# JoshuaLim007/VoxelEngine

Hardware: AMD Instinct MI355X
Metric: Mrays/s primary+1-bounce @1080p, 8k×512×8k brickmap; % HBM roofline (higher is better)
Workload: dtype f32

## Files before the change

include/vxrt.h:

```cpp
#ifndef VXRT_H
#define VXRT_H

#include <stddef.h>
#include <stdint.h>

#ifdef __cplusplus
extern "C" {
#endif

#define VXRT_ABI_VERSION 3
#define VXRT_EMPTY_SLOT 0xFFFFFFFFu
#define VXRT_MAX_STEPS 2048

typedef enum vxrt_status {
    VXRT_OK = 0,
    VXRT_ERR_INVALID = -1,
    VXRT_ERR_HIP = -2,
    VXRT_ERR_NO_WORLD = -3,
    VXRT_ERR_NOMEM = -4
} vxrt_status;

typedef struct vxrt_ctx vxrt_ctx;

int vxrt_abi_version(void);
// ... 318 lines not shown
    int32_t bounce_all_hits;
    int32_t bounce_depth;
    int32_t ortho;
    int64_t frame_number;
    int32_t strip_rows, strip_count, strip_index;
    int32_t compact;
    int32_t collect_stats;
    int32_t tile_schedule;
    float *d_color_aov;
    int64_t *d_hit_aov;
    const uint32_t *d_tile_order;
    void *stream;
    float *d_accum;
    int32_t accum_reset;
    int32_t reserved_;
} vxrt_render_flags;

void vxrt_render_flags_default(vxrt_render_flags *flags);
int vxrt_render(vxrt_ctx *ctx, uint32_t width, uint32_t height, void *d_fb, const float origin[3],
                const float fwd[3], const float up[3], const float right[3], const vxrt_render_flags *flags);
typedef struct vxrt_view {
    void *d_fb;
    float origin[3], fwd[3], up[3], right[3];
    int64_t frame_number;
    float *d_color_aov;
    int64_t *d_hit_aov;
} vxrt_view;
int vxrt_render_views(vxrt_ctx *ctx, uint32_t width, uint32_t height, uint32_t n_views, const vxrt_view *views,
                      const vxrt_render_flags *flags);
int vxrt_kernel_for_launch(const vxrt_ctx *ctx, uint32_t width, uint32_t height, const vxrt_render_flags *flags, uint32_t nviews);
int vxrt_render_specialisation(const vxrt_ctx *ctx, uint32_t width, uint32_t height, const vxrt_render_flags *flags, uint32_t nviews);
uint32_t vxrt_compact_rows(uint32_t height, int32_t strip_rows, int32_t strip_count, int32_t strip_index);
int vxrt_frame_stats_get(vxrt_ctx *ctx, vxrt_frame_stats *out);
int vxrt_deinterleave_strips(vxrt_ctx *ctx, uint32_t width, uint32_t height, int32_t strip_rows,
                             int32_t strip_count, const void *d_shards, uint64_t shard_stride_bytes,
                             void *d_fb, void *stream);
int vxrt_deinterleave_views(vxrt_ctx *ctx, uint32_t width, uint32_t height, int32_t strip_rows, int32_t strip_count,
                            const void *d_shards, uint64_t shard_stride_bytes, uint64_t view_stride_bytes,
                            uint32_t n_views, void *d_fb, uint64_t fb_stride_bytes, void *stream);

typedef struct vxrt_denoise_params {
    uint32_t struct_size;
    int32_t iterations;
    float color_scale;
    int32_t reserved_;
} vxrt_denoise_params;
int vxrt_frame_guides(vxrt_ctx *ctx, uint32_t W, uint32_t H, const float origin[3], const float fwd[3], const float up[3],
                      const float right[3], int32_t ortho, const int64_t *d_hit_aov, uint32_t *d_keys, void *stream);
uint64_t vxrt_denoise_workspace_bytes(uint32_t W, uint32_t H);
int vxrt_denoise_frame(vxrt_ctx *ctx, uint32_t W, uint32_t H, const float *d_color_in , const uint32_t *d_keys,
                       const vxrt_denoise_params *params, void *d_work, float *d_color_out ,
                       void *d_fb_or_null , void *stream);

typedef struct vxrt_history { float r, g, b, n; } vxrt_history;
typedef struct vxrt_camera_pose { float origin[3], fwd[3], up[3], right[3]; } vxrt_camera_pose;
typedef struct vxrt_reproject_params {
    uint32_t struct_size;
    int32_t ortho;
    int32_t max_history;
    int32_t reserved_;
    vxrt_camera_pose cur, prev;
} vxrt_reproject_params;
typedef struct vxrt_reproject_summary { uint32_t hit, reused, offscreen, rejected; } vxrt_reproject_summary;
int vxrt_reproject_frame(vxrt_ctx *ctx, uint32_t W, uint32_t H, const float *d_color_in, const uint32_t *d_keys,
                         const vxrt_history *d_hist_in_or_null, const uint32_t *d_keys_prev_or_null,
                         const vxrt_reproject_params *params, vxrt_history *d_hist_out,
// ... 36 lines not shown
```

voxelengine_amd/_native.py:

```python
from __future__ import annotations

import ctypes as C
import os

from . import build as _build

EMPTY_SLOT = 0xFFFFFFFF
MAX_STEPS = 2048
GEN_HASH_HEIGHTFIELD, GEN_PERLIN_REF, GEN_INT_TERRAIN = 0, 1, 2
MODE_SHADED, MODE_DEBUG = 0, 1

EXPORTS = [
    "vxrt_abi_version", "vxrt_create", "vxrt_destroy", "vxrt_last_error", "vxrt_synchronize", "vxrt_set_kernel_variant", "vxrt_kernel_for_launch",
    "vxrt_render_specialisation",
    "vxrt_has_experiments", "vxrt_set_persistent_waves_per_cu", "vxrt_debug_guard_pretend_no_slack",
    "vxrt_upload_world", "vxrt_build_world_procedural", "vxrt_world_info_get", "vxrt_download_world",
    "vxrt_save_world", "vxrt_load_world", "vxrt_world_file_info",
    "vxrt_set_environment", "vxrt_set_fov", "vxrt_set_ortho_window_size", "vxrt_get_directions",
    "vxrt_render_flags_default", "vxrt_render", "vxrt_render_views", "vxrt_compact_rows", "vxrt_frame_stats_get",
    "vxrt_deinterleave_strips", "vxrt_deinterleave_views", "vxrt_trace_batch", "vxrt_trace_batch_host",
    "vxrt_set_batch_max_steps", "vxrt_stream_open", "vxrt_stream_focus", "vxrt_stream_resident", "vxrt_stream_close",
    "vxrt_edit_voxels", "vxrt_edit_reserve",
    "vxrt_region_words", "vxrt_read_region", "vxrt_read_region_host", "vxrt_edit_stamps",
    "vxrt_move_boxes", "vxrt_overlap_boxes", "vxrt_move_boxes_host", "vxrt_overlap_boxes_host",
    "vxrt_islands_workspace_bytes", "vxrt_find_islands", "vxrt_find_islands_host",
    "vxrt_place_pieces", "vxrt_place_pieces_host",
    "vxrt_orientation_rotation", "vxrt_orientation_compose", "vxrt_orientation_inverse", "vxrt_orientation_dims",
    "vxrt_orientation_voxel", "vxrt_orientation_is_rotation", "vxrt_transform_stamp", "vxrt_transform_stamp_host",
    "vxrt_nav_workspace_bytes", "vxrt_nav_field", "vxrt_nav_paths", "vxrt_nav_field_host",
    "vxrt_distance_workspace_bytes", "vxrt_distance_field", "vxrt_distance_field_host",
    "vxrt_voxelize_workspace_bytes", "vxrt_voxelize_mesh", "vxrt_voxelize_mesh_host",
    "vxrt_surface_workspace_bytes", "vxrt_extract_surface", "vxrt_extract_surface_host",
    "vxrt_lod_workspace_bytes", "vxrt_downsample_region", "vxrt_downsample_region_host",
    "vxrt_light_workspace_bytes", "vxrt_light_field", "vxrt_light_field_host",
    "vxrt_rule_workspace_bytes", "vxrt_apply_rule", "vxrt_apply_rule_host",
    "vxrt_frame_guides", "vxrt_denoise_workspace_bytes", "vxrt_denoise_frame", "vxrt_reproject_frame", "vxrt_light_frame",
]
EDIT_BOX, EDIT_SPHERE = 0, 1
EDIT_MAX_OPS = 1024
STAMP_REPLACE, STAMP_UNION, STAMP_SUBTRACT = 0, 1, 2
BODY_MAX_EXTENT, BODY_MAX_DELTA = 64, 64
BODY_BLOCKED_X, BODY_BLOCKED_Y, BODY_BLOCKED_Z, BODY_INVALID = 1, 2, 4, 8
ISLAND_ANCHOR_X_LO, ISLAND_ANCHOR_X_HI, ISLAND_ANCHOR_Y_LO, ISLAND_ANCHOR_Y_HI = 0x01, 0x02, 0x04, 0x08
ISLAND_ANCHOR_Z_LO, ISLAND_ANCHOR_Z_HI, ISLAND_ANCHOR_FACES, ISLAND_ANCHOR_FLOOR = 0x10, 0x20, 0x3F, 0x40
PLACE_MAX_PIECES, PLACE_MAX_DIM, PLACE_MAX_VOXELS, PLACE_MAX_DIST = 64, 1024, 1 << 24, 4096
PLACED_BLOCKED, PLACED_INVALID = 1, 2
NAV_MAX_GOALS, NAV_NONE, NAV_MAX_STEPS = 4096, 0xFF, 65535
NAV_AT_GOAL, NAV_NO_PATH, NAV_TRUNCATED, NAV_OUTSIDE = 0, 1, 2, 3
DIST_TO_SOLID, DIST_TO_EMPTY, DIST_FAR, DIST_MAX_RADIUS = 0, 1, 0xFFFF, 255
VOX_SURFACE, VOX_SOLID, VOX_FRAC_BITS, VOX_MAX_DIM, VOX_MAX_COORD, VOX_MAX_TRIANGLES = 1, 2, 8, 1024, 1 << 18, 1 << 24
SURF_CAP, SURF_OPEN, SURF_MAX_DIM = 0, 1, 1024
LOD_MAX_SHIFT = 5
# ... 132 lines not shown
    f3 = C.POINTER(C.c_float)
    L.vxrt_abi_version.restype = C.c_int
    L.vxrt_last_error.restype = C.c_char_p
    L.vxrt_create.argtypes = [C.c_int, C.POINTER(C.c_void_p)]
    L.vxrt_destroy.argtypes = [C.c_void_p]
    L.vxrt_synchronize.argtypes = [C.c_void_p]
    L.vxrt_set_kernel_variant.argtypes = [C.c_void_p, C.c_int]
    L.vxrt_has_experiments.restype = C.c_int
    L.vxrt_debug_guard_pretend_no_slack.argtypes = [C.c_void_p, C.c_int]
    L.vxrt_set_persistent_waves_per_cu.argtypes = [C.c_void_p, C.c_int]
    L.vxrt_kernel_for_launch.argtypes = [C.c_void_p, C.c_uint32, C.c_uint32, C.c_void_p, C.c_uint32]
    L.vxrt_kernel_for_launch.restype = C.c_int
    L.vxrt_render_specialisation.argtypes = [C.c_void_p, C.c_uint32, C.c_uint32, C.c_void_p, C.c_uint32]
    L.vxrt_render_specialisation.restype = C.c_int
    L.vxrt_upload_world.argtypes = [C.c_void_p, C.POINTER(WorldDesc)]
    L.vxrt_build_world_procedural.argtypes = [C.c_void_p, C.c_int, C.c_int, C.c_int, C.c_int, C.c_int]
    L.vxrt_world_info_get.argtypes = [C.c_void_p, C.POINTER(WorldInfo)]
    L.vxrt_download_world.argtypes = [C.c_void_p, C.c_void_p, C.c_void_p, C.c_void_p, C.c_void_p]
    L.vxrt_save_world.argtypes = [C.c_void_p, C.c_char_p]
    L.vxrt_load_world.argtypes = [C.c_void_p, C.c_char_p]
    L.vxrt_world_file_info.argtypes = [C.c_char_p, C.POINTER(WorldInfo)]
    L.vxrt_set_environment.argtypes = [C.c_void_p, f3, f3, f3]
    L.vxrt_set_fov.argtypes = [C.c_void_p, C.c_float]
    L.vxrt_set_ortho_window_size.argtypes = [C.c_void_p, C.c_float, C.c_float]
    L.vxrt_get_directions.argtypes = [f3, f3, f3, f3]
    L.vxrt_get_directions.restype = None
    L.vxrt_render_flags_default.argtypes = [C.POINTER(RenderFlags)]
    L.vxrt_render_flags_default.restype = None
    L.vxrt_render.argtypes = [C.c_void_p, C.c_uint32, C.c_uint32, C.c_void_p, f3, f3, f3, f3, C.POINTER(RenderFlags)]
    L.vxrt_render_views.argtypes = [C.c_void_p, C.c_uint32, C.c_uint32, C.c_uint32, C.POINTER(View), C.POINTER(RenderFlags)]
    L.vxrt_compact_rows.argtypes = [C.c_uint32, C.c_int32, C.c_int32, C.c_int32]
    L.vxrt_compact_rows.restype = C.c_uint32
    L.vxrt_frame_stats_get.argtypes = [C.c_void_p, C.POINTER(FrameStats)]
    L.vxrt_deinterleave_strips.argtypes = [C.c_void_p, C.c_uint32, C.c_uint32, C.c_int32, C.c_int32, C.c_void_p,
                                           C.c_uint64, C.c_void_p, C.c_void_p]
    L.vxrt_deinterleave_views.argtypes = [C.c_void_p, C.c_uint32, C.c_uint32, C.c_int32, C.c_int32, C.c_void_p, C.c_uint64,
                                          C.c_uint64, C.c_uint32, C.c_void_p, C.c_uint64, C.c_void_p]
    L.vxrt_trace_batch.argtypes = [C.c_void_p, C.c_void_p, C.c_void_p, C.c_uint64, C.c_void_p, C.c_void_p, C.c_void_p,
                                   C.c_void_p, C.c_void_p, C.POINTER(FrameStats), C.c_void_p]
    L.vxrt_set_batch_max_steps.argtypes = [C.c_void_p, C.c_int32]
    L.vxrt_stream_open.argtypes = [C.c_void_p, C.c_char_p, C.c_uint64]
    L.vxrt_stream_focus.argtypes = [C.c_void_p, f3, C.c_float, C.POINTER(StreamStats)]
    L.vxrt_stream_resident.argtypes = [C.c_void_p, C.c_void_p, C.c_uint64]
    L.vxrt_stream_close.argtypes = [C.c_void_p]
    L.vxrt_edit_voxels.argtypes = [C.c_void_p, C.POINTER(EditOp), C.c_uint32, C.POINTER(EditStats)]
    L.vxrt_edit_reserve.argtypes = [C.c_void_p, C.c_uint64]
    L.vxrt_region_words.restype = C.c_uint64
    L.vxrt_region_words.argtypes = [C.POINTER(C.c_int32)]
    L.vxrt_read_region.argtypes = [C.c_void_p, C.POINTER(C.c_int32), C.POINTER(C.c_int32), C.c_void_p, C.c_void_p]
    L.vxrt_read_region_host.argtypes = [C.c_void_p, C.POINTER(C.c_int32), C.POINTER(C.c_int32), C.c_void_p]
    L.vxrt_edit_stamps.argtypes = [C.c_void_p, C.POINTER(StampDesc), C.c_uint32, C.POINTER(EditStats)]
    L.vxrt_move_boxes.argtypes = [C.c_void_p, C.c_void_p, C.c_uint64, C.POINTER(C.c_int32), C.c_void_p, C.c_void_p,
                                  C.c_void_p]
    L.vxrt_overlap_boxes.argtypes = [C.c_void_p, C.c_void_p, C.c_uint64, C.c_void_p, C.c_void_p, C.c_void_p]
    L.vxrt_move_boxes_host.argtypes = [C.c_void_p, C.c_void_p, C.c_uint64, C.POINTER(C.c_int32), C.c_void_p, C.c_void_p]
    L.vxrt_overlap_boxes_host.argtypes = [C.c_void_p, C.c_void_p, C.c_uint64, C.c_void_p, C.c_void_p]
    L.vxrt_islands_workspace_bytes.restype = C.c_uint64
    L.vxrt_islands_workspace_bytes.argtypes = [C.POINTER(C.c_int32)]
    L.vxrt_find_islands.argtypes = [C.c_void_p, C.POINTER(C.c_int32), C.POINTER(C.c_int32), C.c_uint32, C.c_void_p, C.c_void_p,
                                    C.c_void_p, C.c_void_p, C.c_uint32, C.c_void_p, C.c_void_p]
    L.vxrt_find_islands_host.argtypes = [C.c_void_p, C.POINTER(C.c_int32), C.POINTER(C.c_int32), C.c_uint32, C.c_void_p,
                                         C.c_void_p, C.c_void_p, C.c_uint32, C.c_void_p]
    L.vxrt_place_pieces.argtypes = [C.c_void_p, C.POINTER(PieceDesc), C.c_uint32, C.c_void_p, C.c_uint64, C.c_void_p, C.c_void_p]
    L.vxrt_place_pieces_host.argtypes = [C.c_void_p, C.POINTER(PieceDesc), C.c_uint32, C.c_void_p, C.c_uint64, C.c_void_p]
    po, i3 = C.POINTER(OrientationDesc), C.POINTER(C.c_int32)
    L.vxrt_orientation_rotation.argtypes = [C.c_int, C.c_int, po]
# ... 76 lines not shown
```

voxelengine_amd/csrc/vxrt_api.hip:

```cpp
#include "vxrt_host.hpp"

#include <algorithm>
#include <cmath>
#include <cstdio>
#include <cstdlib>
#include <cstring>
#include <new>
#include <utility>

static thread_local std::string g_last_error = "";

int vxrt::fail(int code, const std::string& msg)
{
    g_last_error = msg;
    return code;
}

namespace vxrt {

void abandon_world(vxrt_ctx* c)
{
    stream_drop(c);
    if (c->coarse_alloc) (void)hipFree(c->coarse_alloc);
    if (c->d_meta) (void)hipFree(c->d_meta);
// ... 785 lines not shown
    VX_HIP(hipDeviceSynchronize());
    unsigned long long now[vxrt::kStatCount] = {}, h[vxrt::kStatCount];
    std::vector<unsigned long long> rows((size_t)vxrt::kStatRows * vxrt::kStatRowStride);
    VX_HIP(hipMemcpy(rows.data(), c->d_stats, rows.size() * sizeof(unsigned long long), hipMemcpyDeviceToHost));
    for (unsigned r = 0; r < vxrt::kStatRows; ++r)
        for (int i = 0; i < vxrt::kStatCount; ++i)
            now[i] += rows[(size_t)r * vxrt::kStatRowStride + i];
    for (int i = 0; i < vxrt::kStatCount; ++i) {
        h[i] = now[i] - c->stats_base[i];
        c->stats_base[i] = now[i];
    }
    out->primary_rays = h[vxrt::kStatPrimary];
    out->shadow_rays = h[vxrt::kStatShadow];
    out->bounce_rays = h[vxrt::kStatBounce];
    out->primary_hits = h[vxrt::kStatPrimaryHits];
    out->coarse_probes = h[vxrt::kStatCoarseProbes];
    out->brick_entries = h[vxrt::kStatBrickEntries];
    out->fine_probes = h[vxrt::kStatFineProbes];
    out->dbg[0] = h[vxrt::kStatDbgIters];
    out->dbg[1] = h[vxrt::kStatDbgWalkLanes];
    out->dbg[2] = h[vxrt::kStatDbgEndRuns];
    out->dbg[3] = h[vxrt::kStatDbgBoxRuns];
    out->dbg[4] = h[vxrt::kStatDbgNextRuns];
    out->dbg[5] = h[vxrt::kStatDbgEndLanes];
    out->dbg[6] = h[vxrt::kStatDbgBoxLanes];
    out->dbg[7] = h[vxrt::kStatDbgNextLanes];
    out->dbg[8] = h[vxrt::kStatDbgLifetime];
    out->dbg[9] = h[vxrt::kStatDbgDrained];
    out->dbg[10] = h[vxrt::kStatDbgNextTicks];
    out->dbg[11] = h[vxrt::kStatDbgParkTicks];
    out->dbg[12] = h[vxrt::kStatDbgEndShadow];
    out->guard_slack_loads = h[vxrt::kStatGuardSlack];
    out->guard_stray_loads = h[vxrt::kStatGuardStray];
#ifdef VXRT_EXPERIMENTS
    if (getenv("VXRT_PRINT_COSTART"))
        fprintf(stderr, "vxrt: rounds with the end-of-walk and the ray-finished phase %llu, with walk starts from both %llu, of %llu rounds\n",
                h[vxrt::kStatDbgCoRuns], h[vxrt::kStatDbgCoStarts], h[vxrt::kStatDbgIters]);
#endif
    return VXRT_OK;
}

int vxrt_deinterleave_strips(vxrt_ctx* c, uint32_t width, uint32_t height, int32_t strip_rows, int32_t strip_count,
                             const void* d_shards, uint64_t shard_stride_bytes, void* d_fb, void* stream)
{
    if (!c || !d_shards || !d_fb)
        return fail(VXRT_ERR_INVALID, "NULL argument");
    if (width % 4 != 0 || shard_stride_bytes % 16 != 0 || strip_rows <= 0 || strip_count <= 0)
        return fail(VXRT_ERR_INVALID, "width must be a multiple of 4 pixels and the shard stride of 16 bytes");
    VX_HIP(hipSetDevice(c->device));
    vxrt::launch_deinterleave(d_shards, shard_stride_bytes, d_fb, width, height, (uint32_t)strip_rows,
                              (uint32_t)strip_count, (hipStream_t)stream);
    VX_HIP(hipGetLastError());
    return VXRT_OK;
}

int vxrt_deinterleave_views(vxrt_ctx* c, uint32_t width, uint32_t height, int32_t strip_rows, int32_t strip_count,
                            const void* d_shards, uint64_t shard_stride_bytes, uint64_t view_stride_bytes, uint32_t n_views,
                            void* d_fb, uint64_t fb_stride_bytes, void* stream)
{
    if (!c || !d_shards || !d_fb)
        return fail(VXRT_ERR_INVALID, "NULL argument");
    if (width % 4 != 0 || shard_stride_bytes % 16 != 0 || view_stride_bytes % 16 != 0 || fb_stride_bytes % 16 != 0 ||
        strip_rows <= 0 || strip_count <= 0)
        return fail(VXRT_ERR_INVALID, "width must be a multiple of 4 pixels and the strides of 16 bytes");
    if (n_views > 65535u)
        return fail(VXRT_ERR_INVALID, "too many views");
    VX_HIP(hipSetDevice(c->device));
    vxrt::launch_deinterleave(d_shards, shard_stride_bytes, d_fb, width, height, (uint32_t)strip_rows, (uint32_t)strip_count,
                              (hipStream_t)stream, n_views, view_stride_bytes, fb_stride_bytes);
    VX_HIP(hipGetLastError());
    return VXRT_OK;
}
// ... 80 lines not shown
```

voxelengine_amd/csrc/vxrt_host.hpp:

```cpp
#pragma once

#include "vxrt_kernels.hpp"
#include "vxrt_region.hpp"

#include <atomic>
#include <set>
#include <string>
#include <vector>

namespace vxrt { int fail(int code, const std::string& msg); }
using vxrt::fail;

#define VX_HIP(call)                                                                                   \
    do {                                                                                               \
        hipError_t e_ = (call);                                                                        \
        if (e_ != hipSuccess)                                                                          \
            return fail(VXRT_ERR_HIP, std::string(#call) + ": " + hipGetErrorString(e_));              \
    } while (0)

struct vxrt_ctx {
    int device = 0;
    bool has_world = false;
    vxrt::WorldView view{};
    uint32_t* d_coarse = nullptr;
    void* coarse_alloc = nullptr;
    void* pool_alloc = nullptr;
    uint2* d_meta = nullptr;
    uint32_t* d_pool = nullptr;
    uint64_t ncells = 0, nslots = 0, pool_capacity_slots = 0;
    uint64_t coarse_alloc_bytes = 0, pool_alloc_bytes = 0;
    bool guard_no_slack = false;
    float light_dir[3] = {0, 0, 0};
    float light_color[3] = {0, 0, 0};
    float ambient[3] = {0, 0, 0};
    float fov = 90.0f;
    float ortho[2] = {10.0f, 10.0f};
    uint32_t frame_counter = 0;
    int kernel_variant = 4;
    unsigned persistent_waves = 4096;
    unsigned cus = 256;
    unsigned long long* d_stats = nullptr;
    unsigned int* d_queues = nullptr;
    unsigned long long stats_base[vxrt::kStatCount] = {};
    std::atomic<unsigned> launch_seq{0};
    hipEvent_t counter_busy[64] = {};
    vxrt::ViewArgs* d_views = nullptr;
    std::atomic<unsigned> view_seq{0};
    hipEvent_t views_busy[16] = {};
    int batch_max_steps = vxrt::kMaxSteps;
    struct StreamState* stream = nullptr;
    std::set<uint32_t> free_slots;
    bool edited = false;
    struct DevBuf {
        void* p = nullptr;
        size_t bytes = 0;
        hipError_t reserve(size_t n)
        {
            if (n <= bytes)
                return hipSuccess;
            (void)hipFree(p);
            p = nullptr;
            bytes = 0;
            hipError_t e = hipMalloc(&p, n);
            if (e == hipSuccess)
                bytes = n;
            return e;
        }
        void release() { (void)hipFree(p); p = nullptr; bytes = 0; }
    } edit_in, edit_scratch, edit_out, edit_plan;
};
constexpr unsigned kViewSlots = 16;
constexpr unsigned kTileCounterRing = 64;
static_assert(kTileCounterRing == sizeof(vxrt_ctx::counter_busy) / sizeof(hipEvent_t), "ring size");
static_assert(kViewSlots == sizeof(vxrt_ctx::views_busy) / sizeof(hipEvent_t), "ring size");

namespace vxrt {
// ... 99 lines not shown
```

voxelengine_amd/csrc/vxrt_kernels.hpp:

```cpp
#pragma once

#include "vxrt_device.hpp"

namespace vxrt {

enum StatSlot {
    kStatPrimary = 0,
    kStatShadow,
    kStatBounce,
    kStatPrimaryHits,
    kStatCoarseProbes,
    kStatBrickEntries,
    kStatFineProbes,
    kStatDbgIters,
    kStatDbgWalkLanes,
    kStatDbgEndRuns,
    kStatDbgBoxRuns,
    kStatDbgNextRuns,
    kStatDbgEndLanes,
    kStatDbgBoxLanes,
    kStatDbgNextLanes,
    kStatDbgLifetime,
    kStatDbgDrained,
    kStatDbgNextTicks,
    kStatDbgParkTicks,
    kStatGuardSlack,
    kStatGuardStray,
    kStatDbgCoRuns,
    kStatDbgCoStarts,
    kStatDbgEndShadow,
    kStatCount
};

#ifndef VXRT_STAT_ROWS
#define VXRT_STAT_ROWS 64
#endif
constexpr unsigned kStatRows = VXRT_STAT_ROWS, kStatRowStride = 32;
static_assert(kStatCount <= (int)kStatRowStride, "a row holds every counter");

constexpr unsigned kMaxScheduledTileRows = 512;

struct RenderArgs {
    WorldView W;
    uint32_t width, height;
    uint32_t frame_number;
    uint32_t launch_rows;
    float kx, ky;
    float ortho_x, ortho_y, ratio;
    f3 origin, fwd, up, right;
    f3 light_dir, light_color, ambient;
    int mode, checkerboard, shadow, bounce_samples, bounce_all_hits, ortho;
    int bounce_depth;
    int strip_rows, strip_count, strip_index, compact;
    int strip_shift;
    uint8_t* fb;
    float* color_aov;
    long long* hit_aov;
    unsigned long long* stats;
    unsigned int* tile_counter;
    unsigned int persistent_waves;
    const unsigned int* tile_order;
    unsigned int row_order_n;
    uint16_t row_order[kMaxScheduledTileRows];
// ... 54 lines not shown
```

voxelengine_amd/csrc/vxrt_persist2.hpp:

```cpp
#pragma once

#include "vxrt_camera.hpp"
#include "vxrt_kernels.hpp"
#include "vxrt_pixel_map.hpp"
#include "vxrt_wave2.hpp"

namespace vxrt {

enum : uint32_t { PX_NONE = 0u, PX_PRIMARY = 1u, PX_SHADOW = 2u, PX_BOUNCE = 3u, PX_BOUNCE2 = 4u };

enum : int { PF_STAGE = 0, PF_TX, PF_ROW, PF_POS_X, PF_POS_Y, PF_POS_Z, PF_COL_X, PF_COL_Y, PF_COL_Z, PF_PCODE, PF_PSTEPS, PF_OCCL,
             PF_SAMPLE, PF_PIXEL_FIELDS };
enum : int { WV_COUNTERS = 0, WV_LIGHT_DX = 4, WV_LIGHT_DY, WV_LIGHT_DZ, WV_LIGHT_IVX, WV_LIGHT_IVY, WV_LIGHT_IVZ, WV_LIGHT_DN,
             WV_LIGHT_STEP_X, WV_LIGHT_STEP_Y, WV_LIGHT_STEP_Z, WV_SHADOW_FROM_END, WV_WORDS = 16 };
#ifndef VXRT_NO_KERNARG_RELOAD
#define VXRT_KERNARG_RELOAD 1
#endif
__device__ __forceinline__ const RenderArgs& kernarg_reload(const RenderArgs& in_registers)
{
#ifdef VXRT_KERNARG_RELOAD
    auto* p = (const __attribute__((address_space(4))) RenderArgs*)__builtin_amdgcn_kernarg_segment_ptr();
    asm volatile("" : "+s"(p));
    return *(const RenderArgs*)p;
#else
    return in_registers;
#endif
}

#ifndef VXRT_PERSIST2_OCC
#define VXRT_PERSIST2_OCC 5
#endif
#ifndef VXRT_QUEUE_GRANULE
#define VXRT_QUEUE_GRANULE 4u
#endif
#ifndef VXRT_SUBROUNDS2
#define VXRT_SUBROUNDS2 3
#endif
#ifndef VXRT_VOTE2_NEXT
#define VXRT_VOTE2_NEXT 2
#endif
#ifndef VXRT_VOTE2_END
#define VXRT_VOTE2_END 1
#endif
#ifndef VXRT_VOTE2_BOX
#define VXRT_VOTE2_BOX 2
#endif
#ifdef VXRT_VOTE2_ABS_BOX
__device__ __forceinline__ bool vote2(int parked, int others, int num, int k)
{
    (void)num;
    return parked >= k || (parked > 0 && others == 0);
}
#else
#define VXRT_VOTE2_ABS_BOX 0
#define VXRT_VOTE2_ABS_END 0
#define VXRT_VOTE2_ABS_NEXT 0
__device__ __forceinline__ bool vote2(int parked, int others, int num, int k)
{
    (void)k;
    return vote_run(parked, others, num);
}
#endif
#define PX_LD_U(f, v) do { if (LDS) v = PX[(f) * 64]; } while (0)
#define PX_ST_U(f, v) do { if (LDS) PX[(f) * 64] = (uint32_t)(v); } while (0)
#define PX_LD_I(f, v) do { if (LDS) v = (int)PX[(f) * 64]; } while (0)
#define PX_LD_F(f, v) do { if (LDS) v = __uint_as_float(PX[(f) * 64]); } while (0)
#define PX_ST_F(f, v) do { if (LDS) PX[(f) * 64] = __float_as_uint(v); } while (0)
#define PX_LD_POS() do { PX_LD_F(PF_POS_X, position.x); PX_LD_F(PF_POS_Y, position.y); PX_LD_F(PF_POS_Z, position.z); } while (0)
#define PX_ST_POS() do { PX_ST_F(PF_POS_X, position.x); PX_ST_F(PF_POS_Y, position.y); PX_ST_F(PF_POS_Z, position.z); } while (0)
#define PX_LD_COL() do { PX_LD_F(PF_COL_X, color.x); PX_LD_F(PF_COL_Y, color.y); PX_LD_F(PF_COL_Z, color.z); } while (0)
#define PX_ST_COL() do { PX_ST_F(PF_COL_X, color.x); PX_ST_F(PF_COL_Y, color.y); PX_ST_F(PF_COL_Z, color.z); } while (0)

template <bool STATS, bool BOUNCE2, bool MULTI, bool WIDE, bool COMMON = false>
__global__ __launch_bounds__(64, VXRT_PERSIST2_OCC) void k_render_persist2(RenderArgs A_kern)
{
    static_assert(!(COMMON && WIDE), "COMMON launches run on ordinary grids");
    using FT = FrameTraits<COMMON>;
    using Tracer = WaveTracerT<WIDE>;
    constexpr bool LDS = true;
    constexpr bool END_SHADOW = !(BOUNCE2 && MULTI) || COMMON;
    constexpr bool BOX_LAST = !(BOUNCE2 && MULTI && !WIDE && !COMMON);
    __shared__ uint32_t cold_block[(CF_TRACER_FIELDS + PF_PIXEL_FIELDS) * 64 + WV_WORDS];
    const WorldView& W = A_kern.W;
    const int lane = threadIdx.x & 63;
    uint32_t* const PX = &cold_block[CF_TRACER_FIELDS * 64 + lane];
    auto lane_view = [&](const RenderArgs& A, uint32_t v) -> LaneView {
        if (MULTI) {
            const ViewArgs& S = A.views[v];
            return LaneView{S.origin, S.fwd, S.up, S.right, S.frame_number, S.fb, S.color_aov, FT::hit_aov(S.hit_aov)};
        }
        return LaneView{A.origin, A.fwd, A.up, A.right, A.frame_number, A.fb, A.color_aov, FT::hit_aov(A.hit_aov)};
    };

    Tracer T;
    T.init(W, &cold_block[lane]);
    uint32_t stage = PX_NONE;
    uint32_t px_tx = 0, px_row = 0;
    f3 position = mk3(0, 0, 0), color = mk3(0, 0, 0);
    uint32_t pcode = 0;
    int p_steps = 0;
    float occl = 0.0f;
    int sample = 0;
    uint32_t n_primary = 0, n_shadow = 0, n_bounce = 0, n_hits = 0;
    PX_ST_U(PF_STAGE, stage);
    uint32_t* const WV = &cold_block[(CF_TRACER_FIELDS + PF_PIXEL_FIELDS) * 64];
    if (lane < 4)
        WV[WV_COUNTERS + lane] = 0u;
    {
        const f3 lu = A_kern.light_unit;
        const float dd = dot3(lu, lu);
        f3 ld = unit3_ordinary(lu, dd);
        const float ex = ld.x == 0 ? kFltEps : ld.x, ey = ld.y == 0 ? kFltEps : ld.y, ez = ld.z == 0 ? kFltEps : ld.z;
        float lix = rcp_rn(ex), liy = rcp_rn(ey), liz = rcp_rn(ez);
        if (!(ordinary(dd) & ordinary(ex) & ordinary(ey) & ordinary(ez))) {
            ld = unit3(lu);
            lix = 1.0f / (ld.x == 0 ? kFltEps : ld.x);
            liy = 1.0f / (ld.y == 0 ? kFltEps : ld.y);
            liz = 1.0f / (ld.z == 0 ? kFltEps : ld.z);
        }
        const bool light_special = !(fabsf(ld.x) >= kMinFastDir && fabsf(ld.y) >= kMinFastDir && fabsf(ld.z) >= kMinFastDir);
        const bool aov = FT::want_hit_aov(A_kern, MULTI);
        if (lane == 0) {
            WV[WV_LIGHT_DX] = __float_as_uint(ld.x);
            WV[WV_LIGHT_DY] = __float_as_uint(ld.y);
            WV[WV_LIGHT_DZ] = __float_as_uint(ld.z);
            WV[WV_LIGHT_IVX] = __float_as_uint(lix);
            WV[WV_LIGHT_IVY] = __float_as_uint(liy);
            WV[WV_LIGHT_IVZ] = __float_as_uint(liz);
            WV[WV_LIGHT_DN] = (ld.x > 0 ? 0u : 1u) | (ld.y > 0 ? 0u : 2u) | (ld.z > 0 ? 0u : 4u);
            WV[WV_LIGHT_STEP_X] = __float_as_uint(A_kern.light_step.x);
            WV[WV_LIGHT_STEP_Y] = __float_as_uint(A_kern.light_step.y);
            WV[WV_LIGHT_STEP_Z] = __float_as_uint(A_kern.light_step.z);
            WV[WV_SHADOW_FROM_END] = (END_SHADOW && FT::mode(A_kern) == 0 && A_kern.shadow && !light_special && !aov) ? 1u : 0u;
        }
    }

    uint32_t tile = 0, tile_used = 64u, tile_view = 0;
    uint32_t queue_shard = blockIdx.x % kQueueShards;
    bool drained = false;
    unsigned long long dg_iters = 0, dg_walk = 0, dg_drain = 0;
    unsigned int dg_runs[3] = {0, 0, 0}, dg_lanes[3] = {0, 0, 0};
    const unsigned long long dg_t0 = STATS ? wall_clock64() : 0ull;
    unsigned long long dg_next_ticks = 0, dg_park_ticks = 0;
    unsigned long long dg_co_runs = 0, dg_co_starts = 0;
    unsigned long long dg_end_shadow = 0;
#ifdef VXRT_TAIL_DEBUG
    unsigned long long px_t0 = 0;
#endif


    auto store_pixel = [&](const RenderArgs& A, const PixelCoords& pc, const LaneView& V, f3 origin, bool hit, f3 normal, f3 pos, f3 shaded) {
        PixelSink sink{A, pc.out_row, V.fb, V.color_aov};
        const int Wd = (int)A.width, Hd = (int)A.height;
        if (hit) {
            if (FT::mode(A) == 1) {
                f3 dv = pos - origin;
                float dist = sqrtf(dot3(dv, dv));
                const float wrap = (float)(1.0 + 1e-6);
                f3 hp = mk3(fmodf(pos.x / 128.0f, wrap), fmodf(pos.y / 128.0f, wrap), fmodf(pos.z / 128.0f, wrap));
                if (pc.x < (Wd >> 1) && pc.y < (Hd >> 1))
                    sink.put(pc.x, pc.y, normal);
                else if (pc.x >= (Wd >> 1) && pc.y < (Hd >> 1))
                    sink.put(pc.x, pc.y, hp);
                else if (pc.x < (Wd >> 1)) {
                } else
                    sink.put(pc.x, pc.y, mk3(dist * 0.01f, 0, 0));
            } else {
                if (!MULTI && FT::accum(A))
                    shaded = accumulate_color(A, pc.out_row, pc.x, shaded);
                const float tx = shaded.x + 1.0f, ty = shaded.y + 1.0f, tz = shaded.z + 1.0f;
                f3 c = mk3(div_rn(shaded.x, tx, rcp_rn(tx)), div_rn(shaded.y, ty, rcp_rn(ty)), div_rn(shaded.z, tz, rcp_rn(tz)));
                const bool plain = !(((shaded.x == 0.0f) | ordinary(shaded.x)) & ((shaded.y == 0.0f) | ordinary(shaded.y)) &
                                     ((shaded.z == 0.0f) | ordinary(shaded.z)) & ordinary(tx) & ordinary(ty) & ordinary(tz));
                if (__ballot(plain) != 0ull)
                    c = mk3(shaded.x / (shaded.x + 1.0f), shaded.y / (shaded.y + 1.0f), shaded.z / (shaded.z + 1.0f));
                c = mk3(lo(hi(c.x, 0), 1), lo(hi(c.y, 0), 1), lo(hi(c.z, 0), 1));
                sink.put(pc.x, pc.y, c);
            }
// ... 29 lines not shown
                    PX[PF_POS_Y * 64] = __float_as_uint(at.y);
                    PX[PF_POS_Z * 64] = __float_as_uint(at.z);
                    PX[PF_COL_X * 64] = 0u;
                    PX[PF_COL_Y * 64] = 0u;
                    PX[PF_COL_Z * 64] = 0u;
                    PX[PF_STAGE * 64] = PX_SHADOW;
                    Tr.cold[CF_RAY_CODES * 64] = (uint32_t)kMaxSteps << 7;
                    Tr.cold[CF_START_X * 64] = __float_as_uint(s0.x);
                    Tr.cold[CF_START_Y * 64] = __float_as_uint(s0.y);
                    Tr.cold[CF_START_Z * 64] = __float_as_uint(s0.z);
                    Tr.cold[CF_LAST_CI * 64] = 0xFFFFFFFFu;
                    Tr.cold[CF_TOTAL * 64] = 0u;
                    Tr.d = mk3(__uint_as_float(WV[WV_LIGHT_DX]), __uint_as_float(WV[WV_LIGHT_DY]), __uint_as_float(WV[WV_LIGHT_DZ]));
                    Tr.ivx = __uint_as_float(WV[WV_LIGHT_IVX]);
                    Tr.ivy = __uint_as_float(WV[WV_LIGHT_IVY]);
                    Tr.ivz = __uint_as_float(WV[WV_LIGHT_IVZ]);
                    Tr.dn = WV[WV_LIGHT_DN];
                    Tr.special = false;
                    Tr.st = ST_WALK;
                    go = true;
                }
            }
        }
        const lanemask_t launched = __ballot(go);
        const uint32_t n = (uint32_t)__popcll(launched);
        if (lane == 0) {
            WV[WV_COUNTERS + 1] += n;
            WV[WV_COUNTERS + 3] += n;
        }
        if (STATS)
            dg_end_shadow += n;
        return launched;
    };

    for (;;) {
        const unsigned long long m_walk = __ballot(T.st == ST_WALK);
        const unsigned long long m_box = __ballot(T.st == ST_BOX);
        const unsigned long long m_end = __ballot(waits_for_end(T.st));
        const unsigned long long m_next = __ballot(T.st == ST_DONE);
        if ((m_walk | m_box | m_end | m_next) == 0ull)
            break;
        const int n_walk = __popcll(m_walk), n_box = __popcll(m_box), n_end = __popcll(m_end), n_next = __popcll(m_next);
        if (STATS) {
            dg_iters += 1;
            dg_walk += (unsigned long long)n_walk;
            dg_drain += drained ? 1ull : 0ull;
        }

        int c_walk = n_walk, c_box = n_box, c_end = n_end, c_next = n_next;
        bool dg_end_ran = false, dg_end_restarted = false;
        if (!BOX_LAST && vote2(c_box, c_walk, VXRT_VOTE2_BOX, VXRT_VOTE2_ABS_BOX)) {
            if (STATS) {
                dg_runs[2] += 1u;
                dg_lanes[2] += (unsigned)c_box;
                dg_park_ticks -= wall_clock64();
            }
            T.template phase_box<STATS>(W);
            if (STATS)
                dg_park_ticks += wall_clock64();
            c_box = 0;
            c_walk = __popcll(__ballot(T.st == ST_WALK));
            c_end = __popcll(__ballot(waits_for_end(T.st)));
        }
        if (vote2(c_end, c_walk + c_box, VXRT_VOTE2_END, VXRT_VOTE2_ABS_END)) {
            if (STATS) {
                dg_runs[1] += 1u;
                dg_lanes[1] += (unsigned)c_end;
                dg_park_ticks -= wall_clock64();
            }
            if constexpr (END_SHADOW)
                T.template phase_end_deferred<STATS>(W, shadow_from_end);
            else
                T.template phase_end_deferred<STATS>(W);
            if (STATS)
                dg_park_ticks += wall_clock64();
            c_end = 0;
            c_walk = __popcll(__ballot(T.st == ST_WALK));
            if (STATS) {
                dg_end_ran = true;
                dg_end_restarted = T.pend_m != 0ull;
            }
            c_next = __popcll(__ballot(T.st == ST_DONE));
        }
        if (vote2(c_next, c_walk + c_box + c_end, VXRT_VOTE2_NEXT, VXRT_VOTE2_ABS_NEXT)) {
            if (STATS) {
                dg_runs[0] += 1u;
                dg_lanes[0] += (unsigned)c_next;
                dg_next_ticks -= wall_clock64();
            }
            const RenderArgs& A = kernarg_reload(A_kern);
            const uint32_t ntx = (A.width + 7u) / 8u, nty = (A.launch_rows + 7u) / 8u, ntiles = ntx * nty;
            const f3 L = A.light_dir;
            const f3 sray = A.light_unit;
            PX_LD_U(PF_STAGE, stage);
            PX_LD_U(PF_TX, px_tx);
            PX_LD_U(PF_ROW, px_row);
            bool launch = false;
            bool c_hit = false, c_shadow = false, c_bounce = false;
            f3 l_origin = mk3(0, 0, 0), l_dir = mk3(1, 0, 0);
            int l_max = kMaxSteps;
            if (T.st == ST_DONE && stage != PX_NONE) {
                const LaneView V = lane_view(A, MULTI ? px_row >> 16 : 0u);
                const PixelCoords pc = pixel_coords<COMMON>(A, V.frame_number, px_tx, MULTI ? px_row & 0xFFFFu : px_row);
                const f3 origin = camera_origin<FT>(A, V, pc.x, pc.y);
// ... 241 lines not shown
    }
    const unsigned long long s0 = n_primary, s1 = n_shadow, s2 = n_bounce, s3 = n_hits;
    unsigned long long* const stats = A_kern.stats ? stats_row_of<kStatRows, kStatRowStride>(A_kern.stats, blockIdx.x) : nullptr;
    if (lane == 0 && stats) {
        atomicAdd(&stats[kStatPrimary], s0);
        atomicAdd(&stats[kStatShadow], s1);
        atomicAdd(&stats[kStatBounce], s2);
        atomicAdd(&stats[kStatPrimaryHits], s3);
    }
    if (STATS) {
        const unsigned long long p0 = wave_sum(T.cnt.coarse_probes), p1 = wave_sum(T.cnt.brick_entries), p2 = wave_sum(T.cnt.fine_probes);
        const unsigned long long g0 = wave_sum(T.cnt.slack_loads), g1 = wave_sum(T.cnt.stray_loads);
        if (lane == 0 && stats) {
            atomicAdd(&stats[kStatCoarseProbes], p0);
            atomicAdd(&stats[kStatBrickEntries], p1);
            atomicAdd(&stats[kStatFineProbes], p2);
            atomicAdd(&stats[kStatGuardSlack], g0);
            atomicAdd(&stats[kStatGuardStray], g1);
            atomicAdd(&stats[kStatDbgIters], dg_iters);
            atomicAdd(&stats[kStatDbgWalkLanes], dg_walk);
            atomicAdd(&stats[kStatDbgNextRuns], (unsigned long long)dg_runs[0]);
            atomicAdd(&stats[kStatDbgEndRuns], (unsigned long long)dg_runs[1]);
            atomicAdd(&stats[kStatDbgBoxRuns], (unsigned long long)dg_runs[2]);
            atomicAdd(&stats[kStatDbgNextLanes], (unsigned long long)dg_lanes[0]);
            atomicAdd(&stats[kStatDbgEndLanes], (unsigned long long)dg_lanes[1]);
            atomicAdd(&stats[kStatDbgBoxLanes], (unsigned long long)dg_lanes[2]);
            atomicAdd(&stats[kStatDbgLifetime], wall_clock64() - dg_t0);
            atomicAdd(&stats[kStatDbgDrained], dg_drain);
            atomicAdd(&stats[kStatDbgNextTicks], dg_next_ticks);
            atomicAdd(&stats[kStatDbgParkTicks], dg_park_ticks);
            atomicAdd(&stats[kStatDbgCoRuns], dg_co_runs);
            atomicAdd(&stats[kStatDbgCoStarts], dg_co_starts);
            atomicAdd(&stats[kStatDbgEndShadow], dg_end_shadow);
        }
    }
}
#undef PX_LD_U
#undef PX_ST_U
#undef PX_LD_I
#undef PX_LD_F
#undef PX_ST_F
#undef PX_LD_POS
#undef PX_ST_POS
#undef PX_LD_COL
#undef PX_ST_COL

}
```

voxelengine_amd/csrc/vxrt_wave2.hpp:

```cpp
#pragma once

#include "vxrt_device.hpp"
#include <type_traits>
#ifdef VXRT_HOST_DEBUG
#include <cstdio>
#include <cstdlib>
#endif

namespace vxrt {

enum : uint32_t { ST_WALK = 0u, ST_BOX = 1u, ST_END = 2u, ST_ENDHIT = 3u, ST_DONE = 4u, ST_IDLE = 5u };
__device__ __forceinline__ bool waits_for_end(uint32_t st) { return (st | 1u) == 3u; }
#ifndef VXRT_PROBE_GD
#define VXRT_PROBE_GD 0
#endif
#ifdef VXRT_HOST_CHECK
inline unsigned long long& host_unsuspected_exits() { static unsigned long long n = 0; return n; }
#endif

__device__ __forceinline__ f3 normal_decode(uint32_t c)
{
    float v = (c & 4u) ? -1.0f : 1.0f;
    uint32_t a = c & 3u;
    return mk3(a == 1u ? v : 0.0f, a == 2u ? v : 0.0f, a == 3u ? v : 0.0f);
// ... 298 lines not shown
        const float dd = dot3(ray, ray);
        d = unit3_ordinary(ray, dd);
        const float ex = d.x == 0 ? kFltEps : d.x, ey = d.y == 0 ? kFltEps : d.y, ez = d.z == 0 ? kFltEps : d.z;
        ivx = rcp_rn(ex);
        ivy = rcp_rn(ey);
        ivz = rcp_rn(ez);
        if (__ballot(!(ordinary(dd) & ordinary(ex) & ordinary(ey) & ordinary(ez))) != 0ull) {
            d = unit3(ray);
            ivx = 1.0f / (d.x == 0 ? kFltEps : d.x);
            ivy = 1.0f / (d.y == 0 ? kFltEps : d.y);
            ivz = 1.0f / (d.z == 0 ? kFltEps : d.z);
        }
        f3 s0 = mk3(origin.x * W.inv_f, origin.y * W.inv_f, origin.z * W.inv_f);
        uint32_t ec = 0u;
        if (!(s0.x >= 0 && s0.y >= 0 && s0.z >= 0 && s0.x < (float)W.cx && s0.y < (float)W.cy && s0.z < (float)W.cz)) {
            const float e = (float)1e-6;
            f3 p;
            uint32_t c;
            if (slab(s0, mk3(e, e, e), mk3(W.wmax_x, W.wmax_y, W.wmax_z), p, c)) {
                s0 = p;
                ec = c;
            }
        }
        cold[CF_RAY_CODES * 64] = ec | ((uint32_t)max_steps_ << 7);
        cold[CF_START_X * 64] = __float_as_uint(s0.x);
        cold[CF_START_Y * 64] = __float_as_uint(s0.y);
        cold[CF_START_Z * 64] = __float_as_uint(s0.z);
        cold[CF_LAST_CI * 64] = 0xFFFFFFFFu;
        cold[CF_TOTAL * 64] = 0u;
        special = !(fabsf(d.x) >= kMinFastDir && fabsf(d.y) >= kMinFastDir && fabsf(d.z) >= kMinFastDir) ||
                  __float_as_uint(s0.x) == 0x80000000u || __float_as_uint(s0.y) == 0x80000000u || __float_as_uint(s0.z) == 0x80000000u;
        dn = (d.x > 0 ? 0u : 1u) | (d.y > 0 ? 0u : 2u) | (d.z > 0 ? 0u : 4u);
        st = ST_WALK;
    }
    __device__ __forceinline__ void after_begin_ray(bool launched) { fine_m &= ~__ballot(launched); }
    __device__ __forceinline__ void after_begin_ray_deferred(bool launched)
    {
        const lanemask_t m = __ballot(launched);
        fine_m &= ~m;
        pend_m |= m;
    }

    __device__ __forceinline__ f3 cross_of(const WorldView& W, bool fine, uint32_t before, uint32_t dec, float t) const
    {
        int bx, by, bz;
        cells_of(W, fine, before, bx, by, bz);
        const bool on_x = dec == kRemDecX, on_y = dec == kRemDecY, on_z = dec == kRemDecZ;
        float face_x = (float)(bx + (d.x > 0 ? 1 : 0)), face_y = (float)(by + (d.y > 0 ? 1 : 0)), face_z = (float)(bz + (d.z > 0 ? 1 : 0));
        float lin_x = ws.x + (t * d.x), lin_y = ws.y + (t * d.y), lin_z = ws.z + (t * d.z);
        pin(face_x), pin(face_y), pin(face_z), pin(lin_x), pin(lin_y), pin(lin_z);
        return mk3(on_x ? face_x : lin_x, on_y ? face_y : lin_y, on_z ? face_z : lin_z);
    }

    __device__ __forceinline__ void walk_on(const WorldView& W, bool is_fine, bool lin_inside)
    {
        const bool single = t_hi == -kInf;
        if (__ballot(single) == 0ull)
            return;
        int x, y, z;
        cells_of(W, is_fine, rem, x, y, z);
        const int dmx = is_fine ? W.f : W.cx, dmy = is_fine ? W.f : W.cy, dmz = is_fine ? W.f : W.cz;
        const int row = is_fine ? W.f_row : W.c_row, slice = is_fine ? W.f_slice : W.c_slice;
        const uint32_t exact = cell_index(min(x, dmx - 1), min(y, dmy - 1), min(z, dmz - 1), row, dmz) + (uint32_t)slice;
        idx = single ? exact : idx;
        const bool pending = x == dmx || y == dmy || z == dmz;
        t_hi = (single && !pending && lin_inside) ? t_hi_real : t_hi;
// ... 447 lines not shown
```

voxelengine_amd/engine.py:

```python
from __future__ import annotations

import ctypes as C
import os
from dataclasses import dataclass, field
from typing import NamedTuple

import numpy as np

from . import _native as N


def _f3(v):
    return (C.c_float * 3)(*[float(x) for x in v])


def GetDirections(euler):
    f, u, r = (C.c_float * 3)(), (C.c_float * 3)(), (C.c_float * 3)()
    N.load().vxrt_get_directions(_f3(euler), f, u, r)
    return (np.array(f[:], np.float32), np.array(u[:], np.float32), np.array(r[:], np.float32))


def tile_schedule(width: int, frame_rows, fwd, up, right, fov_deg: float = 90.0, height: int | None = None):
    frame_rows = np.asarray(list(frame_rows), np.int64)
    H = int(height if height is not None else (frame_rows.max() + 1 if frame_rows.size else 1))
# ... 822 lines not shown
    def _flags(self, opts: RenderOptions | None, stream: int | None) -> "N.RenderFlags":
        o = opts or RenderOptions()
        fl = N.RenderFlags()
        self._L.vxrt_render_flags_default(C.byref(fl))
        fl.mode, fl.checkerboard, fl.shadow = int(o.mode), int(o.checkerboard), int(o.shadow)
        fl.bounce_samples, fl.bounce_all_hits, fl.ortho = int(o.bounce_samples), int(o.bounce_all_hits), int(o.ortho)
        fl.frame_number = int(o.frame_number)
        fl.strip_rows, fl.strip_count, fl.strip_index = int(o.strip_rows), int(o.strip_count), int(o.strip_index)
        fl.compact, fl.collect_stats = int(o.compact), int(o.collect_stats)
        fl.tile_schedule = int(o.tile_schedule)
        fl.bounce_depth = int(o.bounce_depth)
        fl.stream = _stream(stream)
        return fl

    def RenderViews(self, width: int, height: int, views, opts: RenderOptions | None = None,
                    stream: int | None = None) -> None:
        fl = self._flags(opts, stream)
        if opts is not None and opts.extra.get("accum") is not None:
            fl.d_accum = _ptr(opts.extra["accum"])
        arr = (N.View * len(views))()
        for dst, v in zip(arr, views):
            dst.d_fb = _ptr(v["fb"])
            dst.origin, dst.fwd, dst.up, dst.right = _f3(v["origin"]), _f3(v["fwd"]), _f3(v["up"]), _f3(v["right"])
            dst.frame_number = int(v.get("frame_number", fl.frame_number))
            dst.d_color_aov = _ptr(v.get("color_aov"))
            dst.d_hit_aov = _ptr(v.get("hit_aov"))
        N.check(self._L.vxrt_render_views(self._h, width, height, len(views), arr, C.byref(fl)))

    def frame_stats(self) -> "N.FrameStats":
        st = N.FrameStats()
        N.check(self._L.vxrt_frame_stats_get(self._h, C.byref(st)))
        return st

    def deinterleave_strips(self, width, height, strip_rows, strip_count, d_shards, shard_stride_bytes, d_fb,
                            stream: int | None = None) -> None:
        N.check(self._L.vxrt_deinterleave_strips(self._h, width, height, strip_rows, strip_count, _ptr(d_shards),
                                                 int(shard_stride_bytes), _ptr(d_fb), _stream(stream)))

    def deinterleave_views(self, width, height, strip_rows, strip_count, d_shards, shard_stride_bytes, view_stride_bytes,
                           n_views, d_fb, fb_stride_bytes, stream: int | None = None) -> None:
        N.check(self._L.vxrt_deinterleave_views(self._h, width, height, strip_rows, strip_count, _ptr(d_shards),
                                                int(shard_stride_bytes), int(view_stride_bytes), int(n_views), _ptr(d_fb),
                                                int(fb_stride_bytes), _stream(stream)))

    def set_batch_max_steps(self, max_steps: int) -> None:
        N.check(self._L.vxrt_set_batch_max_steps(self._h, int(max_steps)))

    def Raytrace(self, origins, dirs, want_stats: bool = False):
        o = np.ascontiguousarray(origins, np.float32).reshape(-1, 3)
        d = np.ascontiguousarray(dirs, np.float32).reshape(-1, 3)
        n = o.shape[0]
        pos = np.empty((n, 3), np.float32)
        nrm = np.empty((n, 3), np.float32)
        steps = np.empty(n, np.int32)
        hit = np.empty(n, np.uint8)
        vox = np.empty(n, np.int64)
        st = N.FrameStats()
        N.check(self._L.vxrt_trace_batch_host(self._h, o.ctypes.data, d.ctypes.data, n, pos.ctypes.data,
                                              nrm.ctypes.data, steps.ctypes.data, hit.ctypes.data, vox.ctypes.data,
                                              C.byref(st) if want_stats else None))
        valid = np.isfinite(pos).all(axis=1)
        with np.errstate(invalid="ignore"):
            dist = np.sqrt(((o - pos) ** 2).sum(axis=1, dtype=np.float32))
        return dict(hitPoint=pos, normal=nrm, steps=steps, valid=valid, distance=dist, hit=hit, voxel=vox,
                    stats=st if want_stats else None)

# ... 770 lines not shown
```

Baseline: 9591.

## Launch bounce rays directly from end-of-walk hook in persistent kernel

Adds an end-of-walk hook that starts the bounce ray for lanes finishing their shadow stage inside the same wave step, instead of waiting for the normal refill path. It precomputes the per-normal shadowed colors in LDS and adds a fast begin-ray routine for rays starting inside the grid. The aim is fewer idle lanes and fewer scheduler round trips between shadow and bounce stages. It costs extra LDS, more code in the hot loop, and new counters exposed through an API.

```diff
diff --git a/include/vxrt.h b/include/vxrt.h
--- a/include/vxrt.h
+++ b/include/vxrt.h
@@ -374,6 +374,7 @@
 int vxrt_render_specialisation(const vxrt_ctx *ctx, uint32_t width, uint32_t height, const vxrt_render_flags *flags, uint32_t nviews);
 uint32_t vxrt_compact_rows(uint32_t height, int32_t strip_rows, int32_t strip_count, int32_t strip_index);
 int vxrt_frame_stats_get(vxrt_ctx *ctx, vxrt_frame_stats *out);
+int vxrt_loop_counters_get(vxrt_ctx *ctx, uint64_t *out, int32_t capacity);
 int vxrt_deinterleave_strips(vxrt_ctx *ctx, uint32_t width, uint32_t height, int32_t strip_rows,
                              int32_t strip_count, const void *d_shards, uint64_t shard_stride_bytes,
                              void *d_fb, void *stream);
diff --git a/voxelengine_amd/_native.py b/voxelengine_amd/_native.py
--- a/voxelengine_amd/_native.py
+++ b/voxelengine_amd/_native.py
@@ -18,6 +18,7 @@
     "vxrt_save_world", "vxrt_load_world", "vxrt_world_file_info",
     "vxrt_set_environment", "vxrt_set_fov", "vxrt_set_ortho_window_size", "vxrt_get_directions",
     "vxrt_render_flags_default", "vxrt_render", "vxrt_render_views", "vxrt_compact_rows", "vxrt_frame_stats_get",
+    "vxrt_loop_counters_get",
     "vxrt_deinterleave_strips", "vxrt_deinterleave_views", "vxrt_trace_batch", "vxrt_trace_batch_host",
     "vxrt_set_batch_max_steps", "vxrt_stream_open", "vxrt_stream_focus", "vxrt_stream_resident", "vxrt_stream_close",
     "vxrt_edit_voxels", "vxrt_edit_reserve",
@@ -216,6 +217,7 @@
     L.vxrt_compact_rows.argtypes = [C.c_uint32, C.c_int32, C.c_int32, C.c_int32]
     L.vxrt_compact_rows.restype = C.c_uint32
     L.vxrt_frame_stats_get.argtypes = [C.c_void_p, C.POINTER(FrameStats)]
+    L.vxrt_loop_counters_get.argtypes = [C.c_void_p, C.POINTER(C.c_uint64), C.c_int32]
     L.vxrt_deinterleave_strips.argtypes = [C.c_void_p, C.c_uint32, C.c_uint32, C.c_int32, C.c_int32, C.c_void_p,
                                            C.c_uint64, C.c_void_p, C.c_void_p]
     L.vxrt_deinterleave_views.argtypes = [C.c_void_p, C.c_uint32, C.c_uint32, C.c_int32, C.c_int32, C.c_void_p, C.c_uint64,
diff --git a/voxelengine_amd/csrc/vxrt_api.hip b/voxelengine_amd/csrc/vxrt_api.hip
--- a/voxelengine_amd/csrc/vxrt_api.hip
+++ b/voxelengine_amd/csrc/vxrt_api.hip
@@ -841,12 +841,20 @@
     out->dbg[12] = h[vxrt::kStatDbgEndShadow];
     out->guard_slack_loads = h[vxrt::kStatGuardSlack];
     out->guard_stray_loads = h[vxrt::kStatGuardStray];
-#ifdef VXRT_EXPERIMENTS
-    if (getenv("VXRT_PRINT_COSTART"))
-        fprintf(stderr, "vxrt: rounds with the end-of-walk and the ray-finished phase %llu, with walk starts from both %llu, of %llu rounds\n",
-                h[vxrt::kStatDbgCoRuns], h[vxrt::kStatDbgCoStarts], h[vxrt::kStatDbgIters]);
-#endif
-    return VXRT_OK;
+    c->loop_counters[0] = h[vxrt::kStatDbgCoRuns];
+    c->loop_counters[1] = h[vxrt::kStatDbgCoStarts];
+    c->loop_counters[2] = h[vxrt::kStatDbgEndBounce];
+    return VXRT_OK;
+}
+
+int vxrt_loop_counters_get(vxrt_ctx* c, uint64_t* out, int32_t capacity)
+{
+    if (!c || !out || capacity < 0)
+        return fail(VXRT_ERR_INVALID, "NULL argument or negative capacity");
+    const int32_t n = capacity < 3 ? capacity : 3;
+    for (int32_t i = 0; i < n; ++i)
+        out[i] = c->loop_counters[i];
+    return 3;
 }
 
 int vxrt_deinterleave_strips(vxrt_ctx* c, uint32_t width, uint32_t height, int32_t strip_rows, int32_t strip_count,
diff --git a/voxelengine_amd/csrc/vxrt_host.hpp b/voxelengine_amd/csrc/vxrt_host.hpp
--- a/voxelengine_amd/csrc/vxrt_host.hpp
+++ b/voxelengine_amd/csrc/vxrt_host.hpp
@@ -42,6 +42,7 @@
     unsigned long long* d_stats = nullptr;
     unsigned int* d_queues = nullptr;
     unsigned long long stats_base[vxrt::kStatCount] = {};
+    unsigned long long loop_counters[3] = {};
     std::atomic<unsigned> launch_seq{0};
     hipEvent_t counter_busy[64] = {};
     vxrt::ViewArgs* d_views = nullptr;
diff --git a/voxelengine_amd/csrc/vxrt_kernels.hpp b/voxelengine_amd/csrc/vxrt_kernels.hpp
--- a/voxelengine_amd/csrc/vxrt_kernels.hpp
+++ b/voxelengine_amd/csrc/vxrt_kernels.hpp
@@ -29,6 +29,7 @@
     kStatDbgCoRuns,
     kStatDbgCoStarts,
     kStatDbgEndShadow,
+    kStatDbgEndBounce,
     kStatCount
 };
 
diff --git a/voxelengine_amd/csrc/vxrt_persist2.hpp b/voxelengine_amd/csrc/vxrt_persist2.hpp
--- a/voxelengine_amd/csrc/vxrt_persist2.hpp
+++ b/voxelengine_amd/csrc/vxrt_persist2.hpp
@@ -12,7 +12,8 @@
 enum : int { PF_STAGE = 0, PF_TX, PF_ROW, PF_POS_X, PF_POS_Y, PF_POS_Z, PF_COL_X, PF_COL_Y, PF_COL_Z, PF_PCODE, PF_PSTEPS, PF_OCCL,
              PF_SAMPLE, PF_PIXEL_FIELDS };
 enum : int { WV_COUNTERS = 0, WV_LIGHT_DX = 4, WV_LIGHT_DY, WV_LIGHT_DZ, WV_LIGHT_IVX, WV_LIGHT_IVY, WV_LIGHT_IVZ, WV_LIGHT_DN,
-             WV_LIGHT_STEP_X, WV_LIGHT_STEP_Y, WV_LIGHT_STEP_Z, WV_SHADOW_FROM_END, WV_WORDS = 16 };
+             WV_LIGHT_STEP_X, WV_LIGHT_STEP_Y, WV_LIGHT_STEP_Z, WV_SHADOW_FROM_END, WV_BOUNCE_FROM_END, WV_SHADOWED_COL = 16,
+             WV_WORDS = WV_SHADOWED_COL + 24 };
 #ifndef VXRT_NO_KERNARG_RELOAD
 #define VXRT_KERNARG_RELOAD 1
 #endif
@@ -79,6 +80,7 @@
     using Tracer = WaveTracerT<WIDE>;
     constexpr bool LDS = true;
     constexpr bool END_SHADOW = !(BOUNCE2 && MULTI) || COMMON;
+    constexpr bool END_BOUNCE = END_SHADOW && !BOUNCE2;
     constexpr bool BOX_LAST = !(BOUNCE2 && MULTI && !WIDE && !COMMON);
     __shared__ uint32_t cold_block[(CF_TRACER_FIELDS + PF_PIXEL_FIELDS) * 64 + WV_WORDS];
     const WorldView& W = A_kern.W;
@@ -133,6 +135,25 @@
             WV[WV_LIGHT_STEP_Z] = __float_as_uint(A_kern.light_step.z);
             WV[WV_SHADOW_FROM_END] = (END_SHADOW && FT::mode(A_kern) == 0 && A_kern.shadow && !light_special && !aov) ? 1u : 0u;
         }
+        if constexpr (END_BOUNCE) {
+            const f3 L = A_kern.light_dir;
+            const uint32_t exps = 0x7F800000u;
+            const bool finite = (__float_as_uint(L.x) & exps) != exps && (__float_as_uint(L.y) & exps) != exps && (__float_as_uint(L.z) & exps) != exps;
+            const f3 pn = normal_decode((uint32_t)lane & 7u);
+            const f3 normal = mk3(-pn.x, -pn.y, -pn.z);
+            const float l_dot = hi(dot3(normal, L), 0) * (float)0;
+            const f3 diffuse = A_kern.light_color * l_dot;
+            const float up_dot = normal.x * 0.0f + normal.y * 1.0f + normal.z * 0.0f;
+            const float t = (float)((double)up_dot * 0.5 + 0.5);
+            const f3 shadowed_col = diffuse + A_kern.ambient * (0.25f + t * (1.0f - 0.25f));
+            if (lane < 8) {
+                WV[WV_SHADOWED_COL + lane] = __float_as_uint(shadowed_col.x);
+                WV[WV_SHADOWED_COL + 8 + lane] = __float_as_uint(shadowed_col.y);
+                WV[WV_SHADOWED_COL + 16 + lane] = __float_as_uint(shadowed_col.z);
+            }
+            if (lane == 0)
+                WV[WV_BOUNCE_FROM_END] = (FT::mode(A_kern) == 0 && A_kern.shadow && A_kern.bounce_samples > 0 && finite && !light_special && !aov) ? 1u : 0u;
+        }
     }
 
     uint32_t tile = 0, tile_used = 64u, tile_view = 0;
@@ -144,6 +165,7 @@
     unsigned long long dg_next_ticks = 0, dg_park_ticks = 0;
     unsigned long long dg_co_runs = 0, dg_co_starts = 0;
     unsigned long long dg_end_shadow = 0;
+    unsigned long long dg_end_bounce = 0;
 #ifdef VXRT_TAIL_DEBUG
     unsigned long long px_t0 = 0;
 #endif
@@ -239,6 +261,57 @@
             dg_end_shadow += n;
         return launched;
     };
+    auto bounce_from_end = [&](Tracer& Tr, const lanemask_t ended) -> lanemask_t {
+        if (WV[WV_BOUNCE_FROM_END] == 0u)
+            return 0ull;
+        const lanemask_t mine = __ballot(lane_test(ended) && PX[PF_STAGE * 64] == PX_SHADOW);
+        if (mine == 0ull)
+            return 0ull;
+        bool go = false;
+        if (lane_test(mine)) {
+            const RenderArgs& A = kernarg_reload(A_kern);
+            const uint32_t tx = PX[PF_TX * 64], row = PX[PF_ROW * 64];
+            const PixelCoords pc = pixel_coords<COMMON>(A, 0u, tx, MULTI ? row & 0xFFFFu : row);
+            const uint32_t seed = pc.ty * A.width + pc.tx;
+            const uint32_t frame_number = MULTI ? A.views[row >> 16].frame_number : A.frame_number;
+            const uint32_t si = seed + (frame_number + 1u) * 1000u;
+            float two = 2.0f;
+            pin(two);
+            f3 sd = mk3(random_float(si) * two - 1, random_float(si * 10u) * two - 1, random_float(si * 100u) * two - 1);
+            const float sdd = dot3(sd, sd);
+            sd = unit3_ordinary(sd, sdd);
+            const uint32_t code = PX[PF_PCODE * 64];
+            const f3 pn = normal_decode(code);
+            const f3 bn = mk3(-pn.x, -pn.y, -pn.z);
+            if (dot3(sd, bn) < 0)
+                sd = reflect3(sd, bn);
+            const f3 bo = mk3(__uint_as_float(PX[PF_POS_X * 64]), __uint_as_float(PX[PF_POS_Y * 64]), __uint_as_float(PX[PF_POS_Z * 64]));
+            if (ordinary(sdd) && Tr.begin_ray_inside_fast(W, bo + bn * 0.01f, sd, 8)) {
+                PX[PF_COL_X * 64] = WV[WV_SHADOWED_COL + (code & 7u)];
+                PX[PF_COL_Y * 64] = WV[WV_SHADOWED_COL + 8 + (code & 7u)];
+                PX[PF_COL_Z * 64] = WV[WV_SHADOWED_COL + 16 + (code & 7u)];
+                PX[PF_OCCL * 64] = 0u;
+                PX[PF_SAMPLE * 64] = 0u;
+                PX[PF_STAGE * 64] = PX_BOUNCE;
+                go = true;
+            }
+        }
+        const lanemask_t launched = __ballot(go);
+        const uint32_t n = (uint32_t)__popcll(launched);
+        if (lane == 0)
+            WV[WV_COUNTERS + 2] += n;
+        if (STATS)
+            dg_end_bounce += n;
+        return launched;
+    };
+    auto end_hook = [&](Tracer& Tr, const lanemask_t ended) -> lanemask_t {
+        lanemask_t launched = shadow_from_end(Tr, ended);
+        if constexpr (END_BOUNCE) {
+            if (ended != 0ull)
+                launched |= bounce_from_end(Tr, ended & ~launched);
+        }
+        return launched;
+    };
 
     for (;;) {
         const unsigned long long m_walk = __ballot(T.st == ST_WALK);
@@ -276,7 +349,7 @@
                 dg_park_ticks -= wall_clock64();
             }
             if constexpr (END_SHADOW)
-                T.template phase_end_deferred<STATS>(W, shadow_from_end);
+                T.template phase_end_deferred<STATS>(W, end_hook);
             else
                 T.template phase_end_deferred<STATS>(W);
             if (STATS)
@@ -584,6 +657,7 @@
             atomicAdd(&stats[kStatDbgCoRuns], dg_co_runs);
             atomicAdd(&stats[kStatDbgCoStarts], dg_co_starts);
             atomicAdd(&stats[kStatDbgEndShadow], dg_end_shadow);
+            atomicAdd(&stats[kStatDbgEndBounce], dg_end_bounce);
         }
     }
 }
diff --git a/voxelengine_amd/csrc/vxrt_wave2.hpp b/voxelengine_amd/csrc/vxrt_wave2.hpp
--- a/voxelengine_amd/csrc/vxrt_wave2.hpp
+++ b/voxelengine_amd/csrc/vxrt_wave2.hpp
@@ -354,6 +354,32 @@
                   __float_as_uint(s0.x) == 0x80000000u || __float_as_uint(s0.y) == 0x80000000u || __float_as_uint(s0.z) == 0x80000000u;
         dn = (d.x > 0 ? 0u : 1u) | (d.y > 0 ? 0u : 2u) | (d.z > 0 ? 0u : 4u);
         st = ST_WALK;
+    }
+    __device__ __forceinline__ bool begin_ray_inside_fast(const WorldView& W, f3 origin, f3 ray, int max_steps_)
+    {
+        const float dd = dot3(ray, ray);
+        const f3 u = unit3_ordinary(ray, dd);
+        const float ix = rcp_rn(u.x), iy = rcp_rn(u.y), iz = rcp_rn(u.z);
+        const f3 s0 = mk3(origin.x * W.inv_f, origin.y * W.inv_f, origin.z * W.inv_f);
+        const uint32_t signs = __float_as_uint(s0.x) | __float_as_uint(s0.y) | __float_as_uint(s0.z);
+        const bool ok = ordinary(dd) & (fabsf(u.x) >= kMinFastDir) & (fabsf(u.y) >= kMinFastDir) & (fabsf(u.z) >= kMinFastDir) &
+                        ((int32_t)signs >= 0) & (s0.x < (float)W.cx) & (s0.y < (float)W.cy) & (s0.z < (float)W.cz);
+        if (!ok)
+            return false;
+        d = u;
+        ivx = ix;
+        ivy = iy;
+        ivz = iz;
+        cold[CF_RAY_CODES * 64] = (uint32_t)max_steps_ << 7;
+        cold[CF_START_X * 64] = __float_as_uint(s0.x);
+        cold[CF_START_Y * 64] = __float_as_uint(s0.y);
+        cold[CF_START_Z * 64] = __float_as_uint(s0.z);
+        cold[CF_LAST_CI * 64] = 0xFFFFFFFFu;
+        cold[CF_TOTAL * 64] = 0u;
+        special = false;
+        dn = (u.x > 0 ? 0u : 1u) | (u.y > 0 ? 0u : 2u) | (u.z > 0 ? 0u : 4u);
+        st = ST_WALK;
+        return true;
     }
     __device__ __forceinline__ void after_begin_ray(bool launched) { fine_m &= ~__ballot(launched); }
     __device__ __forceinline__ void after_begin_ray_deferred(bool launched)
diff --git a/voxelengine_amd/engine.py b/voxelengine_amd/engine.py
--- a/voxelengine_amd/engine.py
+++ b/voxelengine_amd/engine.py
@@ -878,6 +878,15 @@
         N.check(self._L.vxrt_frame_stats_get(self._h, C.byref(st)))
         return st
 
+    def loop_counters(self) -> dict:
+        names = ("co_runs", "co_starts", "end_bounce")
+        out = (C.c_uint64 * len(names))()
+        n = self._L.vxrt_loop_counters_get(self._h, out, len(names))
+        if n < 0:
+            N.check(n)
+        assert n == len(names), "vxrt_loop_counters_get reports %d counters" % n
+        return {k: int(out[i]) for i, k in enumerate(names)}
+
     def deinterleave_strips(self, width, height, strip_rows, strip_count, d_shards, shard_stride_bytes, d_fb,
                             stream: int | None = None) -> None:
         N.check(self._L.vxrt_deinterleave_strips(self._h, width, height, strip_rows, strip_count, _ptr(d_shards),
```

Result: faster. 9775, median of 6 (+1.9%).
